# arkworks-rs/marlin

Hardware: NVIDIA H100
Metric: prover_constraints_per_sec (higher is better)
Workload: dtype u32-limb modular integers (Fr 255-bit, Fq 381-bit)

## Files before the change

marlin_b200/csrc/msm.cuh:

```cuda
#pragma once
#include "common.cuh"
#include "curve.cuh"

namespace b2m {

constexpr int MSM_MIN_WINDOW = 8;
constexpr int MSM_BKT_BITS = 24;
constexpr uint32_t MSM_BKT_MASK = (1u << MSM_BKT_BITS) - 1;
constexpr uint32_t MSM_NO_DIGIT = 0xffffffffu;
constexpr int MSM_MAX_BATCH = 8;
constexpr int MSM_MAX_AFFINE_LEVELS = 6;
constexpr size_t MSM_AFFINE_MIN_REFS = (size_t)1 << 23;

template <class Fr, class Fq>
struct MsmJob {
  const Fr* scalars;
  bool mont;
  size_t n;
  size_t base_off;
  const Fr* scalars2;
  size_t n2;
  size_t extra_base;
  const XYZZ<Fq>* extra;
  int n_extra;
  XYZZ<Fq>* out_xyzz;
  Affine<Fq>* out_affine;
  size_t scalar_stride = 1;
};

template <class Fr, class Fq>
struct Msm {
  Ctx* ctx;
  size_t n_srs = 0;
  size_t n_srs_global = 0;
  int tab_rank = 0, tab_world = 1;
  size_t n_extra = 0;
  size_t stride = 0;
  int c = 0, W = 0;
  int affine_levels = Fq::N > 8 ? 3 : 0;
  int affine_ctas_upper = 22;
  int affine_ctas = 4;
  size_t affine_min_refs = MSM_AFFINE_MIN_REFS;
  int affine_map = 1;
  int affine_T = 64;
  int affine_T_upper = 32;
  int acc_ctas_per_sm = 3;
  DBuf<Affine<Fq>> tables;

  static int pick_window(size_t n);
  Msm(Ctx& cx, const Affine<Fq>* powers, size_t n, const Affine<Fq>* host_extra, size_t n_extra_bases, int window_bits,
      bool powers_on_device = false);

  void run(const Fr* scalars, bool mont, size_t n, size_t base_off, const XYZZ<Fq>* extra, int n_extra, XYZZ<Fq>* out_xyzz,
           Affine<Fq>* out_affine);
  void run_batch(const MsmJob<Fr, Fq>* jobs, int nj);
  void run_host(size_t base_off, const uint64_t* scalars, size_t n, uint64_t* out_xy, int* out_is_inf);
  void read_power(size_t i, uint64_t* out_xy);
  static void g1_to_bytes(Ctx& cx, const Affine<Fq>* dev_pts, const uint64_t* host_pts, size_t n, uint8_t* out);
  static void g1_from_bytes(Ctx& cx, const uint8_t* bytes, size_t n, uint64_t* out_xy);
  static void g1_powers_host(Ctx& cx, const uint64_t* g_xy, const uint64_t* beta, size_t n, uint64_t* out);
  static void fixed_base_host(Ctx& cx, const uint64_t* g_xy, const uint64_t* scalars, const uint64_t* beta, size_t first, size_t n, uint64_t* out);
};

}
```

marlin_b200/csrc/msm_affine.cuh:

```cuda
#pragma once
#include "curve.cuh"
#ifdef __CUDACC__
#include "devmem.cuh"
#else
struct uint2 {
  uint32_t x, y;
};
struct uint4 {
  uint32_t x, y, z, w;
};
#endif

namespace b2m {

constexpr uint32_t AFF_BKT_BITS = 24;

template <class Fq>
struct AffLevel {
  const Affine<Fq>* tables;
  size_t table_stride;
  const uint2* sorted;
  const Affine<Fq>* in;
  const uint32_t* off_in;
  const uint32_t* off_out;
  uint32_t B;
  Affine<Fq>* out;
  uint2* out_refs;
  Fq* pref;
  uint4* meta;
  uint32_t T, nthreads;
  uint32_t lane_step;
  Fq* inv;
};

struct AffMap {
  uint32_t o0, step, cnt;
};
template <class Fq>
B2M_HD AffMap aff_map(const AffLevel<Fq>& A, uint32_t t, uint32_t total) {
  AffMap m;
  m.step = A.lane_step;
  uint64_t o0;
  if (A.lane_step == 1) {
    o0 = (uint64_t)t * A.T;
  } else {
    o0 = (uint64_t)(t / A.lane_step) * A.lane_step * A.T + (t % A.lane_step);
  }
  if (o0 >= total) {
    m.o0 = 0;
    m.cnt = 0;
    return m;
  }
  m.o0 = (uint32_t)o0;
  const uint32_t left = (total - m.o0 + m.step - 1) / m.step;
  m.cnt = left < A.T ? left : A.T;
  return m;
}

#if defined(__CUDA_ARCH__)
#define B2M_AFF_LDG(p) ldg_words(p)
#define B2M_AFF_LD(p) ld_words(p)
#define B2M_AFF_ST(p, v) st_words(p, v)
#define B2M_AFF_LDG32(p) __ldg(p)
#else
#define B2M_AFF_LDG(p) (*(p))
#define B2M_AFF_LD(p) (*(p))
#define B2M_AFF_ST(p, v) (*(p) = (v))
#define B2M_AFF_LDG32(p) (*(p))
#endif

B2M_HD uint32_t aff_bucket_of(const uint32_t* off, uint32_t n, uint32_t v) {
  uint32_t lo = 0, hi = n;
  while (hi - lo > 1) {
    uint32_t mid = (lo + hi) >> 1;
    if (B2M_AFF_LDG32(off + mid) <= v) lo = mid; else hi = mid;
  }
  return lo;
}

template <class Fq, bool L0>
B2M_HD void aff_plan_thread(const AffLevel<Fq>& A, uint32_t t) {
  const uint32_t total = B2M_AFF_LDG32(A.off_out + A.B);
  const AffMap mp = aff_map(A, t, total);
  if (!mp.cnt) return;
  uint32_t b = aff_bucket_of(A.off_out, A.B, mp.o0);
  uint32_t b_start = B2M_AFF_LDG32(A.off_out + b), b_end = B2M_AFF_LDG32(A.off_out + b + 1);
  for (uint32_t k = 0; k < mp.cnt; k++) {
    const uint32_t o = mp.o0 + k * mp.step;
    if (o >= b_end) {
      int steps = 0;
      do {
        b++;
        b_end = B2M_AFF_LDG32(A.off_out + b + 1);
      } while (o >= b_end && ++steps < 8);
      if (o >= b_end) {
        b = aff_bucket_of(A.off_out, A.B, o);
        b_end = B2M_AFF_LDG32(A.off_out + b + 1);
      }
      b_start = B2M_AFF_LDG32(A.off_out + b);
    }
    const uint32_t in_start = B2M_AFF_LDG32(A.off_in + b), in_end = B2M_AFF_LDG32(A.off_in + b + 1);
    const uint32_t i0 = in_start + 2u * (o - b_start);
    const bool pair = i0 + 1u < in_end;
    uint4 m;
    if (L0) {
      const uint2 r0 = B2M_AFF_LDG32(A.sorted + i0);
      m.x = (uint32_t)((size_t)(r0.y >> AFF_BKT_BITS) * A.table_stride + (r0.x & 0x7fffffffu)) | (r0.x & 0x80000000u);
      m.y = m.x;
      if (pair) {
        const uint2 r1 = B2M_AFF_LDG32(A.sorted + i0 + 1u);
        m.y = (uint32_t)((size_t)(r1.y >> AFF_BKT_BITS) * A.table_stride + (r1.x & 0x7fffffffu)) | (r1.x & 0x80000000u);
      }
    } else {
      m.x = i0;
      m.y = pair ? i0 + 1u : i0;
    }
    m.z = b;
    m.w = pair ? 1u : 0u;
    A.meta[(size_t)k * A.nthreads + t] = m;
  }
}

template <class Fq>
B2M_HD Fq aff_ldx(const Affine<Fq>* base, uint32_t ref) {
  return B2M_AFF_LDG(&base[ref & 0x7fffffffu].x);
}
template <class Fq>
B2M_HD Affine<Fq> aff_ld(const Affine<Fq>* base, uint32_t ref) {
  const Affine<Fq>* p = base + (ref & 0x7fffffffu);
  Affine<Fq> r;
  r.x = B2M_AFF_LDG(&p->x);
  r.y = B2M_AFF_LDG(&p->y);
  return r;
}
template <class Fq>
B2M_HD Affine<Fq> aff_signed(Affine<Fq> p, uint32_t ref) {
  if (ref >> 31) p.y = p.y.neg();
  return p;
// ... 302 lines not shown
```

marlin_b200/csrc/msm_impl.cuh:

```cuda
#pragma once
#include "msm.cuh"
#include "devmem.cuh"
#include "scan.cuh"
#include "msm_affine.cuh"
#include "comm.cuh"

namespace b2m {

template <class Fq>
__device__ __forceinline__ Affine<Fq> ld_affine(const Affine<Fq>* p) {
  Affine<Fq> r;
  const uint4* q = reinterpret_cast<const uint4*>(p);
  uint32_t* d = reinterpret_cast<uint32_t*>(&r);
#pragma unroll
  for (int i = 0; i < 2 * Fq::N / 4; i++) {
    uint4 v = __ldg(q + i);
    d[4 * i] = v.x; d[4 * i + 1] = v.y; d[4 * i + 2] = v.z; d[4 * i + 3] = v.w;
  }
  return r;
}
template <class Fq> __device__ __noinline__ void g1_add(XYZZ<Fq>& a, const XYZZ<Fq>& b) { a.add(b); }
template <class Fq> __device__ __noinline__ void g1_add_mixed(XYZZ<Fq>& a, const Affine<Fq>& b) { a.add_mixed(b); }
template <class Fq> __device__ __noinline__ void g1_dbl(XYZZ<Fq>& a) { a = a.dbl(); }
template <class Fq> __device__ __noinline__ Fq fq_inverse(const Fq& a) { return a.inverse_fast(); }
template <class Fq> __device__ __noinline__ Affine<Fq> g1_to_affine(const XYZZ<Fq>& p) {
  if (p.is_inf()) return Affine<Fq>::inf();
  Fq izzz = fq_inverse(p.ZZZ);
  Fq izz = (p.ZZ * izzz).sqr();
  return Affine<Fq>{p.X * izz, p.Y * izzz};
}
template <class Fq> __device__ __noinline__ XYZZ<Fq> g1_scalar_mul(const Affine<Fq>& p, const uint32_t* k, int nlimbs) {
  XYZZ<Fq> acc = XYZZ<Fq>::inf();
  bool started = false;
  for (int i = nlimbs - 1; i >= 0; i--) {
    for (int b = 31; b >= 0; b--) {
      if (started) g1_dbl(acc);
      if ((k[i] >> b) & 1u) {
        g1_add_mixed(acc, p);
        started = true;
      }
    }
  }
  return acc;
}

template <class Fq>
__global__ void msm_precompute_kernel(Affine<Fq>* tables, size_t n, int c, int W) {
  size_t i = blockIdx.x * (size_t)blockDim.x + threadIdx.x;
  if (i >= n) return;
  Affine<Fq> cur = ld_affine(tables + i);
  for (int w = 1; w < W; w++) {
    XYZZ<Fq> acc = XYZZ<Fq>::from_affine(cur);
    for (int k = 0; k < c; k++) g1_dbl(acc);
    cur = g1_to_affine(acc);
    st_words(tables + (size_t)w * n + i, cur);
  }
}

template <class Fq>
__global__ void msm_take_residue_kernel(const Affine<Fq>* all, size_t n_loc, int rank, int world, Affine<Fq>* tables) {
  size_t k = blockIdx.x * (size_t)blockDim.x + threadIdx.x;
  if (k >= n_loc) return;
  st_words(tables + k, ld_affine(all + k * (size_t)world + rank));
}

template <class Fr>
__global__ void msm_digits_kernel(const Fr* scalars, size_t sstride, const Fr* scalars2, bool MONT, size_t n, size_t nt, int c, int W,
                                  uint32_t* digits, uint32_t* hist) {
  size_t i = blockIdx.x * (size_t)blockDim.x + threadIdx.x;
  if (i >= nt) return;
  Fr s = i < n ? ld_fr(scalars + i * sstride) : ld_fr(scalars2 + (i - n));
  if (MONT) s = s.to_canonical();
  const uint32_t half = 1u << (c - 1);
  uint32_t carry = 0;
  for (int w = 0; w < W; w++) {
    int bit = w * c;
    int limb = bit >> 5, off = bit & 31;
    uint32_t raw = 0;
    if (limb < Fr::N) {
      raw = s.l[limb] >> off;
      if (off + c > 32 && limb + 1 < Fr::N) raw |= s.l[limb + 1] << (32 - off);
      raw &= (1u << c) - 1;
    }
    uint32_t v = raw + carry;
    uint32_t out;
    if (v > half) {
      uint32_t mag = (1u << c) - v;
      carry = 1;
      out = (mag - 1) | 0x80000000u;
    } else {
      carry = 0;
      out = v ? (v - 1) : MSM_NO_DIGIT;
    }
    digits[(size_t)w * nt + i] = out;
    if (out != MSM_NO_DIGIT) atomicAdd(hist + (out & 0x7fffffffu), 1u);
  }
}


static __global__ void msm_scatter_kernel(const uint32_t* digits, size_t n, size_t nt, size_t base_off, size_t idx2, int W,
                                          uint32_t* cursor, uint2* sorted) {
  size_t i = blockIdx.x * (size_t)blockDim.x + threadIdx.x;
  if (i >= nt) return;
  uint32_t abs_idx = (uint32_t)(i < n ? base_off + i : idx2 + (i - n));
  for (int w = 0; w < W; w++) {
    uint32_t d = digits[(size_t)w * nt + i];
    if (d == MSM_NO_DIGIT) continue;
    uint32_t bkt = d & 0x7fffffffu;
    uint32_t pos = atomicAdd(cursor + bkt, 1u);
    sorted[pos] = make_uint2(abs_idx | (d & 0x80000000u), bkt | ((uint32_t)w << MSM_BKT_BITS));
  }
}

constexpr int MSM_Q = 64;
constexpr int MSM_Q_MIN = 32;
template <class Fq>
__global__ void __launch_bounds__(128)
msm_accumulate_kernel(const Affine<Fq>* __restrict__ tables, size_t table_stride, const uint32_t* __restrict__ offsets,
                      const uint32_t* __restrict__ ends, const uint2* __restrict__ sorted, const uint32_t* __restrict__ total_refs_p,
                      const uint32_t q, XYZZ<Fq>* __restrict__ buckets, XYZZ<Fq>* __restrict__ part_pt,
                      uint32_t* __restrict__ part_bkt) {
  const uint32_t total = *total_refs_p;
  const uint32_t t = blockIdx.x * blockDim.x + threadIdx.x;
  const uint64_t start64 = (uint64_t)t * q;
  uint32_t head_b = MSM_NO_DIGIT, tail_b = MSM_NO_DIGIT;
  if (start64 < total) {
    const uint32_t start = (uint32_t)start64;
    const uint32_t end = (total - start > q) ? start + q : total;
    uint2 rb = __ldg(sorted + start);
    uint32_t ref = rb.x;
    uint32_t cur_b = rb.y & MSM_BKT_MASK;
    uint32_t seg_start = start;
    Affine<Fq> p = ld_affine(tables + (size_t)(rb.y >> MSM_BKT_BITS) * table_stride + (ref & 0x7fffffffu));
    XYZZ<Fq> acc = XYZZ<Fq>::inf();
    for (uint32_t e = start; e < end; e++) {
      Affine<Fq> cur = p;
      const bool neg = ref >> 31;
      uint32_t next_b = cur_b;
      if (e + 1 < end) {
        rb = __ldg(sorted + e + 1);
        ref = rb.x;
        next_b = rb.y & MSM_BKT_MASK;
        p = ld_affine(tables + (size_t)(rb.y >> MSM_BKT_BITS) * table_stride + (ref & 0x7fffffffu));
      }
      acc.add_mixed(cur, neg);
      if (e + 1 == end || next_b != cur_b) {
        const bool whole = (seg_start == offsets[cur_b]) && (e + 1 == ends[cur_b]);
        if (whole) {
          st_words(buckets + cur_b, acc);
        } else if (seg_start == start && head_b == MSM_NO_DIGIT) {
          st_words(part_pt + 2 * (size_t)t, acc);
          head_b = cur_b;
        } else {
          st_words(part_pt + 2 * (size_t)t + 1, acc);
          tail_b = cur_b;
        }
        acc = XYZZ<Fq>::inf();
        seg_start = e + 1;
        cur_b = next_b;
      }
    }
  }
  part_bkt[2 * (size_t)t] = head_b;
  part_bkt[2 * (size_t)t + 1] = tail_b;
}
static __global__ void msm_level_counts_kernel(const uint32_t* off_in, uint32_t B, uint32_t* cnt) {
  uint32_t b = blockIdx.x * blockDim.x + threadIdx.x;
  if (b > B) return;
  cnt[b] = b < B ? (off_in[b + 1] - off_in[b] + 1u) / 2u : 0u;
}
template <class Fq, bool L0>
__global__ void __launch_bounds__(256) msm_affine_plan_kernel(const AffLevel<Fq> A) {
  const uint32_t t = blockIdx.x * blockDim.x + threadIdx.x;
  if (t < A.nthreads) aff_plan_thread<Fq, L0>(A, t);
}
template <class Fq, int MINB, bool PF>
__global__ void __launch_bounds__(128, MINB) msm_affine_level_kernel(const AffLevel<Fq> A, const Affine<Fq>* __restrict__ base) {
  const uint32_t t = blockIdx.x * blockDim.x + threadIdx.x;
  if (t < A.nthreads) aff_level_thread<Fq, PF>(A, base, t);
}

template <class Fq, int MINB, int PHASE, bool PIPE = true>
__global__ void __launch_bounds__(128, MINB) msm_affine_level_sp_kernel(const AffLevel<Fq> A, const Affine<Fq>* __restrict__ base) {
  const uint32_t t = blockIdx.x * blockDim.x + threadIdx.x;
  if (t < A.nthreads) aff_level_thread_sp<Fq, PHASE, PIPE>(A, base, t);
}

template <class Fq>
__device__ __forceinline__ Fq shfl_fq(const Fq& a, int src_lane) {
  Fq r;
#pragma unroll
  for (int i = 0; i < Fq::N; i++) r.l[i] = __shfl_sync(0xffffffffu, a.l[i], src_lane);
  return r;
}
template <class Fq>
__global__ void __launch_bounds__(128) fq_batch_inverse_kernel(Fq* v, size_t n) {
  constexpr int G = 4;
  const size_t t = blockIdx.x * (size_t)blockDim.x + threadIdx.x;
  const int lane = threadIdx.x & 31;
  const size_t i0 = t * G;
  Fq e[G], pre[G];
  Fq run = Fq::one();
#pragma unroll
  for (int k = 0; k < G; k++) {
    e[k] = i0 + k < n ? ld_words(v + i0 + k) : Fq::one();
    pre[k] = run;
    run = run * e[k];
  }
  Fq pin = run, sin = run;
#pragma unroll
  for (int d = 1; d < 32; d <<= 1) {
    const Fq up = shfl_fq(pin, lane - d < 0 ? lane : lane - d);
    const Fq dn = shfl_fq(sin, lane + d > 31 ? lane : lane + d);
    if (lane >= d) pin = pin * up;
    if (lane + d <= 31) sin = sin * dn;
  }
  Fq tinv = Fq::one();
  if (lane == 31) tinv = fq_inverse(pin);
  tinv = shfl_fq(tinv, 31);
  Fq before = shfl_fq(pin, lane == 0 ? 0 : lane - 1), after = shfl_fq(sin, lane == 31 ? 31 : lane + 1);
  if (lane == 0) before = Fq::one();
  if (lane == 31) after = Fq::one();
  Fq inv_run = tinv * before * after;
#pragma unroll
  for (int k = G - 1; k >= 0; k--) {
    const Fq ek = inv_run * pre[k];
    inv_run = inv_run * e[k];
    if (i0 + k < n) st_words(v + i0 + k, ek);
  }
}

struct MsmLongRun {
  uint32_t first, last, bucket;
  uint32_t dst;
};
constexpr uint32_t MSM_RUN_CHUNK = 256;
constexpr uint32_t MSM_RUN_SHORT = 12;
template <class Fq>
__global__ void __launch_bounds__(128)
msm_stitch_kernel(const XYZZ<Fq>* part_pt, const uint32_t* part_bkt, size_t nthreads, const uint32_t q, const uint32_t* offsets,
                  const uint32_t* ends, XYZZ<Fq>* buckets, MsmLongRun* long_runs, MsmLongRun* final_runs, MsmLongRun* short_runs, uint32_t* n_long,
                  uint32_t long_cap, uint32_t chunk_cap) {
  size_t u = blockIdx.x * (size_t)blockDim.x + threadIdx.x;
  if (u >= nthreads) return;
  uint32_t first = 2u * (uint32_t)u + 1u;
  uint32_t b = part_bkt[first];
  if (b == MSM_NO_DIGIT) {
    first = 2u * (uint32_t)u;
    b = part_bkt[first];
    if (b == MSM_NO_DIGIT || offsets[b] != (uint32_t)u * q) return;
  }
  const uint32_t t1 = (ends[b] - 1u) / q;
  const uint32_t last = 2u * t1;
  if (t1 > (uint32_t)u + 1u) {
    const uint32_t nslots = last - first + 1u;
    if (nslots <= MSM_RUN_SHORT) {
      const uint32_t slot = atomicAdd(n_long + 3, 1u);
      if (slot < long_cap) {
        short_runs[slot] = MsmLongRun{first, last, b, MSM_NO_DIGIT};
        return;
      }
    } else if (nslots <= MSM_RUN_CHUNK) {
      const uint32_t slot = atomicAdd(n_long, 1u);
      if (slot < long_cap) {
        long_runs[slot] = MsmLongRun{first, last, b, MSM_NO_DIGIT};
        return;
      }
    } else {
      const uint32_t nch = (nslots + MSM_RUN_CHUNK - 1u) / MSM_RUN_CHUNK;
      const uint32_t c0 = atomicAdd(n_long + 2, nch);
      const uint32_t base = atomicAdd(n_long, nch);
      if (c0 + nch <= chunk_cap && base + nch <= long_cap) {
        for (uint32_t k = 0; k < nch; k++) {
          const uint32_t f = first + k * MSM_RUN_CHUNK;
          const uint32_t l = (last - f >= MSM_RUN_CHUNK) ? f + MSM_RUN_CHUNK - 1u : last;
          long_runs[base + k] = MsmLongRun{f, l, b, c0 + k};
        }
        final_runs[atomicAdd(n_long + 1, 1u)] = MsmLongRun{c0, c0 + nch - 1u, b, MSM_NO_DIGIT};
        return;
      }
      for (uint32_t k = 0; k < nch && base + k < long_cap; k++) long_runs[base + k] = MsmLongRun{1u, 0u, b, MSM_NO_DIGIT};
    }
    XYZZ<Fq> acc = ld_words(part_pt + first);
    for (uint32_t k = first + 1; k <= last; k++)
      if (part_bkt[k] == b) g1_add(acc, ld_words(part_pt + k));
    st_words(buckets + b, acc);
    return;
  }
  XYZZ<Fq> acc = ld_words(part_pt + first);
  g1_add(acc, ld_words(part_pt + last));
  st_words(buckets + b, acc);
}
template <class Fq>
__global__ void __launch_bounds__(128)
msm_stitch_short_kernel(const XYZZ<Fq>* part_pt, const uint32_t* part_bkt, const MsmLongRun* runs, const uint32_t* n_runs, uint32_t cap,
                        XYZZ<Fq>* buckets) {
  uint32_t count = *n_runs;
  if (count > cap) count = cap;
  for (uint32_t r = blockIdx.x * blockDim.x + threadIdx.x; r < count; r += gridDim.x * blockDim.x) {
    const MsmLongRun run = runs[r];
    XYZZ<Fq> acc = ld_words(part_pt + run.first);
    for (uint32_t k = run.first + 1; k <= run.last; k++)
      if (part_bkt[k] == run.bucket) g1_add(acc, ld_words(part_pt + k));
    st_words(buckets + run.bucket, acc);
  }
}
template <class Fq, bool FINAL>
__global__ void __launch_bounds__(128)
msm_stitch_runs_kernel(const XYZZ<Fq>* part_pt, const uint32_t* part_bkt, const MsmLongRun* runs, const uint32_t* n_runs, uint32_t cap,
                       XYZZ<Fq>* buckets, XYZZ<Fq>* chunk_pt) {
  __shared__ uint4 sm_raw[128 * sizeof(XYZZ<Fq>) / 16];
  XYZZ<Fq>* sm = reinterpret_cast<XYZZ<Fq>*>(sm_raw) + (threadIdx.x & ~31u);
  const uint32_t lane = threadIdx.x & 31u;
  uint32_t count = *n_runs;
  if (count > cap) count = cap;
  const uint32_t warps = gridDim.x * (blockDim.x >> 5);
  for (uint32_t r = blockIdx.x * (blockDim.x >> 5) + (threadIdx.x >> 5); r < count; r += warps) {
    const MsmLongRun run = runs[r];
    if (run.first > run.last) continue;
    XYZZ<Fq> acc = XYZZ<Fq>::inf();
    for (uint32_t k = run.first + lane; k <= run.last; k += 32) {
      if (FINAL) g1_add(acc, ld_words(chunk_pt + k));
      else if (part_bkt[k] == run.bucket) g1_add(acc, ld_words(part_pt + k));
    }
    sm[lane] = acc;
    __syncwarp();
    for (uint32_t s2 = 16; s2 >= 1; s2 >>= 1) {
// ... 133 lines not shown
  }
}

template <class Fq>
__global__ void __launch_bounds__(32) msm_combine_kernel(const XYZZ<Fq>* all, int world, int nj, MsmFinishJobs jobs) {
  const int j = blockIdx.x;
  if (threadIdx.x != 0) return;
  XYZZ<Fq> total = XYZZ<Fq>::inf();
  for (int r = 0; r < world; r++) g1_add(total, ld_words(all + (size_t)r * nj + j));
  const XYZZ<Fq>* extra = reinterpret_cast<const XYZZ<Fq>*>(jobs.j[j].extra);
  for (int i = 0; i < jobs.j[j].n_extra; i++) g1_add(total, ld_words(extra + i));
  if (jobs.j[j].out_xyzz) st_words(reinterpret_cast<XYZZ<Fq>*>(jobs.j[j].out_xyzz), total);
  if (jobs.j[j].out_affine) st_words(reinterpret_cast<Affine<Fq>*>(jobs.j[j].out_affine), g1_to_affine(total));
}

constexpr int FB_WIN = 8, FB_WINDOWS = 32, FB_NORM = 16;
template <class Fq>
__global__ void fixed_base_table_kernel(Affine<Fq> g, Affine<Fq>* table) {
  const int t = blockIdx.x * blockDim.x + threadIdx.x;
  if (t >= FB_WINDOWS * 256) return;
  const int k = t >> 8, j = t & 255;
  uint32_t sc[8] = {0, 0, 0, 0, 0, 0, 0, 0};
  sc[k >> 2] = (uint32_t)j << (8 * (k & 3));
  st_words(table + t, j ? g1_to_affine(g1_scalar_mul<Fq>(g, sc, 8)) : Affine<Fq>::inf());
}
template <class Fr, class Fq>
__global__ void __launch_bounds__(128) fixed_base_mul_kernel(const Affine<Fq>* __restrict__ table, const Fr* scalars, Fr beta, size_t first, size_t n,
                                                             XYZZ<Fq>* out) {
  const size_t i = blockIdx.x * (size_t)blockDim.x + threadIdx.x;
  if (i >= n) return;
  const Fr k = scalars ? ld_fr(scalars + i) : beta.pow_u64(first + i).to_canonical();
  XYZZ<Fq> acc = XYZZ<Fq>::inf();
  for (int w = 0; w < FB_WINDOWS && w * FB_WIN < 32 * Fr::N; w++) {
    const uint32_t d = (k.l[w >> 2] >> (8 * (w & 3))) & 255u;
    if (d) g1_add_mixed(acc, ld_affine(table + w * 256 + d));
  }
  st_words(out + i, acc);
}
template <class Fq>
__global__ void __launch_bounds__(128) batch_normalize_kernel(const XYZZ<Fq>* pts, size_t n, Affine<Fq>* out) {
  const size_t t = blockIdx.x * (size_t)blockDim.x + threadIdx.x;
  const size_t i0 = t * FB_NORM;
  if (i0 >= n) return;
  const int cnt = (int)(n - i0 < (size_t)FB_NORM ? n - i0 : FB_NORM);
  Fq pref[FB_NORM];
  Fq run = Fq::one();
  for (int k = 0; k < cnt; k++) {
    const Fq zzz = ld_words(&pts[i0 + k].ZZZ);
    pref[k] = run;
    if (!zzz.is_zero()) run = run * zzz;
  }
  Fq inv = fq_inverse(run);
  for (int k = cnt - 1; k >= 0; k--) {
    const XYZZ<Fq> p = ld_words(pts + i0 + k);
    if (p.is_inf()) {
      st_words(out + i0 + k, Affine<Fq>::inf());
      continue;
    }
    const Fq izzz = inv * pref[k];
    inv = inv * p.ZZZ;
    const Fq izz = (p.ZZ * izzz).sqr();
    st_words(out + i0 + k, Affine<Fq>{p.X * izz, p.Y * izzz});
  }
}

template <class Fq>
__global__ void g1_canonical_kernel(const Affine<Fq>* in, size_t n, Affine<Fq>* out, bool to_bytes) {
  const size_t i = blockIdx.x * (size_t)blockDim.x + threadIdx.x;
  if (i >= n) return;
  Affine<Fq> p = ld_words(in + i);
  if (to_bytes) {
    const bool inf = p.is_inf();
    p.x = p.x.to_canonical();
    p.y = p.y.to_canonical();
    if (inf) p.y.l[Fq::N - 1] |= 1u << 30;
  } else {
    const bool inf = (p.y.l[Fq::N - 1] >> 30) & 1u;
    p.y.l[Fq::N - 1] &= 0x3fffffffu;
    p.x = Fq::from_canonical(p.x);
    p.y = Fq::from_canonical(p.y);
    if (inf) p = Affine<Fq>::inf();
  }
  st_words(out + i, p);
}

template <class Fr, class Fq>
int Msm<Fr, Fq>::pick_window(size_t n) {
  int lg = 0;
  while (((size_t)1 << (lg + 1)) <= n) lg++;
  int c = lg >= 21 ? 20 : (lg >= 17 ? 16 : lg - 1);
  if (c < MSM_MIN_WINDOW) c = MSM_MIN_WINDOW;
  if (c > 20) c = 20;
  auto top_bits = [](int w) {
    const int W = (Fr::Params::BITS + 1 + w - 1) / w;
    return Fr::Params::BITS + 1 - (W - 1) * w;
  };
  if (top_bits(c) < 6) {
    if (c + 1 <= 20 && top_bits(c + 1) >= 6) c = c + 1;
    else if (c - 1 >= MSM_MIN_WINDOW && top_bits(c - 1) >= 6) c = c - 1;
    else if (c - 2 >= MSM_MIN_WINDOW && top_bits(c - 2) >= 6) c = c - 2;
  }
  return c;
}

template <class Fr, class Fq>
Msm<Fr, Fq>::Msm(Ctx& cx, const Affine<Fq>* host_powers, size_t n, const Affine<Fq>* host_extra, size_t n_extra_bases, int window_bits,
                 bool powers_on_device)
    : ctx(&cx), n_extra(n_extra_bases), n_srs_global(n) {
  B2M_REQUIRE(!powers_on_device || cx.world <= 1, B2M_ERR_UNSUPPORTED, "device-resident bases on a multi-GPU context");
  tab_world = cx.world > 1 ? cx.world : 1;
  tab_rank = cx.world > 1 ? cx.rank : 0;
  n_srs = n > (size_t)tab_rank ? (n - tab_rank + tab_world - 1) / tab_world : 0;
  stride = n_srs + n_extra;
  B2M_REQUIRE(n >= 1 && stride < ((size_t)1 << 31), B2M_ERR_INVALID_ARG, "SRS size %zu out of range", n);
  c = window_bits > 0 ? window_bits : pick_window(n / (size_t)tab_world);
  B2M_REQUIRE(c >= MSM_MIN_WINDOW && c <= 24, B2M_ERR_INVALID_ARG, "window bits %d out of range [%d, 24]", c, MSM_MIN_WINDOW);
  W = (Fr::Params::BITS + 1 + c - 1) / c;
  B2M_REQUIRE(W <= 32, B2M_ERR_INVALID_ARG, "too many windows (%d)", W);
  tables = DBuf<Affine<Fq>>(cx, (size_t)W * stride);
  if (powers_on_device) {
    B2M_CUDA(cudaMemcpyAsync(tables.p, host_powers, n * sizeof(Affine<Fq>), cudaMemcpyDeviceToDevice, cx.stream));
  } else if (tab_world == 1) {
    tables.upload(host_powers, n);
  } else if (n_srs) {
    DBuf<Affine<Fq>> all(cx, n);
    all.upload(host_powers, n);
    msm_take_residue_kernel<Fq><<<div_up(n_srs, 256), 256, 0, cx.stream>>>(all.p, n_srs, tab_rank, tab_world, tables.p);
    B2M_CHECK_LAUNCH();
    cx.launches++;
  }
  if (n_extra) B2M_CUDA(cudaMemcpyAsync(tables.p + n_srs, host_extra, n_extra * sizeof(Affine<Fq>), cudaMemcpyHostToDevice, cx.stream));
  if (stride) {
    msm_precompute_kernel<Fq><<<div_up(stride, 128), 128, 0, cx.stream>>>(tables.p, stride, c, W);
    B2M_CHECK_LAUNCH();
    cx.launches++;
  }
  cx.sync();
  B2M_CUDA(cudaOccupancyMaxActiveBlocksPerMultiprocessor(&acc_ctas_per_sm, msm_accumulate_kernel<Fq>, 128, 0));
  if (acc_ctas_per_sm < 1) acc_ctas_per_sm = 1;
  if (const char* e = getenv("B2M_MSM_AFFINE_LEVELS")) affine_levels = atoi(e);
  if (const char* e = getenv("B2M_MSM_AFFINE_T")) affine_T = affine_T_upper = atoi(e);
  if (const char* e = getenv("B2M_MSM_AFFINE_T_UPPER")) affine_T_upper = atoi(e);
  if (const char* e = getenv("B2M_MSM_AFFINE_CTAS")) affine_ctas = atoi(e);
  if (const char* e = getenv("B2M_MSM_AFFINE_CTAS_UPPER")) affine_ctas_upper = atoi(e);
  if (const char* e = getenv("B2M_MSM_AFFINE_MIN_REFS")) affine_min_refs = (size_t)atoll(e);
  if (const char* e = getenv("B2M_MSM_AFFINE_MAP")) affine_map = atoi(e);

  if (affine_levels < 0) affine_levels = 0;
  if (affine_levels > MSM_MAX_AFFINE_LEVELS) affine_levels = MSM_MAX_AFFINE_LEVELS;
  if (affine_T < 1) affine_T = 1;
  if (affine_T > 1024) affine_T = 1024;
  if (affine_T_upper < 1) affine_T_upper = 1;
  if (affine_T_upper > 1024) affine_T_upper = 1024;
}

template <class Fr, class Fq>
void Msm<Fr, Fq>::run(const Fr* scalars, bool mont, size_t n, size_t base_off, const XYZZ<Fq>* extra, int n_extra,
                      XYZZ<Fq>* out_xyzz, Affine<Fq>* out_affine) {
  MsmJob<Fr, Fq> job{scalars, mont, n, base_off, nullptr, 0, 0, extra, n_extra, out_xyzz, out_affine};
  run_batch(&job, 1);
}

template <class Fr, class Fq>
void Msm<Fr, Fq>::run_batch(const MsmJob<Fr, Fq>* jobs_in, int nj) {
  Ctx& cx = *ctx;
  B2M_REQUIRE(nj >= 1 && nj <= MSM_MAX_BATCH, B2M_ERR_INVALID_ARG, "MSM batch of %d jobs", nj);
  MsmJob<Fr, Fq> local[MSM_MAX_BATCH];
  const bool sharded = cx.world > 1;
  B2M_REQUIRE((sharded ? cx.world : 1) == tab_world && (sharded ? cx.rank : 0) == tab_rank, B2M_ERR_INVALID_ARG,
              "this key's tables were built for rank %d of %d; create the SRS after b2m_ctx_attach_comm", tab_rank, tab_world);
  DBuf<XYZZ<Fq>> partial, gathered;
  if (sharded) {
    partial = DBuf<XYZZ<Fq>>(cx, nj);
    gathered = DBuf<XYZZ<Fq>>(cx, (size_t)nj * cx.world);
  }
  for (int j = 0; j < nj; j++) {
    local[j] = jobs_in[j];
    B2M_REQUIRE(jobs_in[j].base_off + jobs_in[j].n <= n_srs_global, B2M_ERR_DEGREE_TOO_LARGE,
                "MSM slice [%zu, %zu) exceeds the SRS (%zu powers)", jobs_in[j].base_off, jobs_in[j].base_off + jobs_in[j].n, n_srs_global);
    if (sharded) {
      const size_t G = (size_t)cx.world, off = jobs_in[j].base_off, n = jobs_in[j].n;
      const size_t skip = ((size_t)cx.rank + G - off % G) % G;
      const size_t cnt = n > skip ? (n - skip + G - 1) / G : 0;
      local[j].scalars = jobs_in[j].scalars + skip;
      local[j].scalar_stride = G;
      local[j].base_off = (off + skip) / G;
      local[j].n = cnt;
      if (cx.rank != 0) { local[j].scalars2 = nullptr; local[j].n2 = 0; }
      local[j].extra = nullptr; local[j].n_extra = 0;
      local[j].out_xyzz = partial.p + j; local[j].out_affine = nullptr;
    }
  }
  const MsmJob<Fr, Fq>* jobs = local;
  size_t max_n = 0;
  for (int j = 0; j < nj; j++) {
    B2M_REQUIRE(jobs[j].n == 0 || jobs[j].base_off + jobs[j].n <= n_srs, B2M_ERR_DEGREE_TOO_LARGE, "MSM slot range [%zu, %zu) exceeds the tables (%zu)",
                jobs[j].base_off, jobs[j].base_off + jobs[j].n, n_srs);
    B2M_REQUIRE(jobs[j].n2 == 0 || jobs[j].extra_base + jobs[j].n2 <= n_extra, B2M_ERR_INVALID_ARG, "extra bases out of range");
    max_n = std::max(max_n, jobs[j].n + jobs[j].n2);
  }
  B2M_REQUIRE((size_t)W * max_n < ((size_t)1 << 32), B2M_ERR_DEGREE_TOO_LARGE, "MSM of %zu pairs x %d windows exceeds 2^32 bucket references", max_n, W);
  MsmFinishJobs fj;
  for (int j = 0; j < nj; j++) fj.j[j] = MsmFinishJob{jobs[j].extra, jobs[j].n_extra, jobs[j].out_xyzz, jobs[j].out_affine};
  auto exchange = [&]() {
    if (!sharded) return;
    size_t spx = cx.span_begin("msm_allgather", (double)nj);
    all_gather_bytes(cx, partial.p, gathered.p, (size_t)nj * sizeof(XYZZ<Fq>));
    MsmFinishJobs oj;
    for (int j = 0; j < nj; j++) oj.j[j] = MsmFinishJob{jobs_in[j].extra, jobs_in[j].n_extra, jobs_in[j].out_xyzz, jobs_in[j].out_affine};
    msm_combine_kernel<Fq><<<nj, 32, 0, cx.stream>>>(gathered.p, cx.world, nj, oj);
    B2M_CHECK_LAUNCH();
    cx.launches++;
    cx.span_end(spx);
  };
  if (max_n == 0) {
    msm_finish_kernel<Fq><<<nj, 64, 0, cx.stream>>>(nullptr, 0, nullptr, 0, 0, fj);
    B2M_CHECK_LAUNCH();
    cx.launches++;
    exchange();
    return;
  }
  const uint32_t B = 1u << (c - 1);
  const int cbits = (c - 1 + 1) / 2, rbits = (c - 1) - cbits;
  const size_t L = (size_t)1 << cbits, R = (size_t)1 << rbits;
  DBuf<XYZZ<Fq>> buckets(cx, (size_t)nj * B);
  {
    const size_t max_refs = (size_t)W * max_n;
    const size_t max_threads = (max_refs + MSM_Q_MIN - 1) / MSM_Q_MIN + 256;
    DBuf<uint32_t> digits[2], hist[2], offsets[2], cursor[2];
    DBuf<uint2> sorted[2];
    const int slots = nj > 1 ? 2 : 1;
    for (int s = 0; s < slots; s++) {
      digits[s] = DBuf<uint32_t>(cx, max_refs); hist[s] = DBuf<uint32_t>(cx, B + 1); offsets[s] = DBuf<uint32_t>(cx, B + 1);
      cursor[s] = DBuf<uint32_t>(cx, B); sorted[s] = DBuf<uint2>(cx, max_refs);
    }
    DBuf<uint32_t> part_bkt(cx, 2 * max_threads), n_long(cx, 4);
    const uint32_t long_cap = 1u << 18;
    const uint32_t chunk_cap = (uint32_t)(4 * max_threads / MSM_RUN_CHUNK + 4);
    DBuf<MsmLongRun> long_runs(cx, long_cap), short_runs(cx, long_cap), final_runs(cx, chunk_cap);
    DBuf<XYZZ<Fq>> chunk_pt(cx, chunk_cap);
    DBuf<XYZZ<Fq>> part_pt(cx, 2 * max_threads);
    const int LV = max_refs >= affine_min_refs ? affine_levels : 0;
    B2M_REQUIRE(LV == 0 || (size_t)W * stride < ((size_t)1 << 31), B2M_ERR_DEGREE_TOO_LARGE,
                "window tables of %d x %zu entries exceed the 31-bit index of the batched-affine plan", W, stride);
    size_t bound[MSM_MAX_AFFINE_LEVELS + 1];
    bound[0] = max_refs;
    for (int l = 1; l <= LV; l++) bound[l] = (bound[l - 1] + B) / 2 + 1;
    DBuf<Affine<Fq>> lvl_pts[2];
    DBuf<uint32_t> lvl_off[2], lvl_cnt;
    DBuf<uint2> lvl_refs;
    DBuf<uint4> lvl_meta;
    DBuf<Fq> lvl_pref, lvl_inv;
    if (LV > 0) {
      lvl_pts[0] = DBuf<Affine<Fq>>(cx, bound[1]);
      if (LV > 1) lvl_pts[1] = DBuf<Affine<Fq>>(cx, bound[2]);
      lvl_off[0] = DBuf<uint32_t>(cx, B + 1); lvl_off[1] = DBuf<uint32_t>(cx, B + 1); lvl_cnt = DBuf<uint32_t>(cx, B + 1);
      lvl_refs = DBuf<uint2>(cx, bound[LV]);
      const size_t T_max = (size_t)std::max(affine_T, affine_T_upper), T_min = (size_t)std::min(affine_T, affine_T_upper);
      const size_t slots_l0 = T_max * ((bound[1] + T_max - 1) / T_max + 128);
      lvl_meta = DBuf<uint4>(cx, slots_l0);
      lvl_pref = DBuf<Fq>(cx, slots_l0);
      lvl_inv = DBuf<Fq>(cx, slots_l0 / T_min + 256);
    }
    buckets.zero();
    cudaEvent_t ev_ready, ev_sorted[MSM_MAX_BATCH], ev_acc[MSM_MAX_BATCH];
    B2M_CUDA(cudaEventCreateWithFlags(&ev_ready, cudaEventDisableTiming));
    for (int j = 0; j < nj; j++) {
      B2M_CUDA(cudaEventCreateWithFlags(&ev_sorted[j], cudaEventDisableTiming));
      B2M_CUDA(cudaEventCreateWithFlags(&ev_acc[j], cudaEventDisableTiming));
    }
    B2M_CUDA(cudaEventRecord(ev_ready, cx.stream));
    B2M_CUDA(cudaStreamWaitEvent(cx.side, ev_ready, 0));
    for (int j = 0; j < nj; j++) {
      const size_t n = jobs[j].n, nt = jobs[j].n + jobs[j].n2;
      const int s = j % slots;
      if (nt == 0) {
        B2M_CUDA(cudaEventRecord(ev_acc[j], cx.stream));
        continue;
      }
      {
        StreamSwap on_side(cx, cx.side);
        if (j >= slots) B2M_CUDA(cudaStreamWaitEvent(cx.side, ev_acc[j - slots], 0));
        hist[s].zero();
        size_t sp0 = cx.span_begin("msm_sort", (double)n);
        msm_digits_kernel<Fr><<<div_up(nt, 256), 256, 0, cx.stream>>>(jobs[j].scalars, jobs[j].scalar_stride, jobs[j].scalars2, jobs[j].mont, n, nt, c, W,
                                                                      digits[s].p, hist[s].p);
        B2M_CHECK_LAUNCH();
        exclusive_scan_u32(cx, hist[s].p, offsets[s].p, B + 1);
        B2M_CUDA(cudaMemcpyAsync(cursor[s].p, offsets[s].p, B * sizeof(uint32_t), cudaMemcpyDeviceToDevice, cx.stream));
        msm_scatter_kernel<<<div_up(nt, 256), 256, 0, cx.stream>>>(digits[s].p, n, nt, jobs[j].base_off, n_srs + jobs[j].extra_base, W,
                                                                    cursor[s].p, sorted[s].p);
        B2M_CHECK_LAUNCH();
        cx.launches += 2;
        cx.span_end(sp0);
        B2M_CUDA(cudaEventRecord(ev_sorted[j], cx.side));
      }
      B2M_CUDA(cudaStreamWaitEvent(cx.stream, ev_sorted[j], 0));
      const Affine<Fq>* src_tables = tables.p;
      size_t src_stride = stride;
      const uint32_t* src_off = offsets[s].p;
      const uint2* src_sorted = sorted[s].p;
      size_t refs = (size_t)W * nt;
      if (LV > 0 && refs >= affine_min_refs) {
        size_t spl = cx.span_begin("msm_affine_levels", (double)n);
        bound[0] = refs;
        for (int l = 1; l <= LV; l++) bound[l] = (bound[l - 1] + B) / 2 + 1;
        const uint32_t* off_in = offsets[s].p;
        for (int l = 0; l < LV; l++) {
          uint32_t* off_out = lvl_off[l & 1].p;
          msm_level_counts_kernel<<<div_up((size_t)B + 1, 256), 256, 0, cx.stream>>>(off_in, B, lvl_cnt.p);
          B2M_CHECK_LAUNCH();
          cx.launches++;
          exclusive_scan_u32(cx, lvl_cnt.p, off_out, (size_t)B + 1);
          const uint32_t lane_step = affine_map ? 32u : 1u;
          const size_t T_l = (size_t)(l == 0 ? affine_T : affine_T_upper);
          const uint32_t nthreads = (uint32_t)(lane_step * ((bound[l + 1] + (size_t)lane_step * T_l - 1) / ((size_t)lane_step * T_l)));
          AffLevel<Fq> A{tables.p, stride, sorted[s].p, l > 0 ? lvl_pts[(l - 1) & 1].p : nullptr, off_in, off_out, B, lvl_pts[l & 1].p,
                         l == LV - 1 ? lvl_refs.p : nullptr, lvl_pref.p, lvl_meta.p, (uint32_t)T_l, nthreads, lane_step, lvl_inv.p};
          if (l == 0)
            msm_affine_plan_kernel<Fq, true><<<div_up(nthreads, 256), 256, 0, cx.stream>>>(A);
          else
            msm_affine_plan_kernel<Fq, false><<<div_up(nthreads, 256), 256, 0, cx.stream>>>(A);
          const Affine<Fq>* base = l == 0 ? tables.p : lvl_pts[(l - 1) & 1].p;
          const unsigned grid = div_up(nthreads, 128);
          const int variant = l == 0 ? affine_ctas : affine_ctas_upper;
          static const char* const lvl_names[MSM_MAX_AFFINE_LEVELS] = {"msm_aff_level0", "msm_aff_level1", "msm_aff_level2", "msm_aff_level3",
                                                                       "msm_aff_level4", "msm_aff_level5"};
          const size_t spk = cx.span_begin(lvl_names[l], (double)n);
          switch (variant) {
            case 3: msm_affine_level_kernel<Fq, 3, true><<<grid, 128, 0, cx.stream>>>(A, base); break;
            case 5: msm_affine_level_kernel<Fq, 5, false><<<grid, 128, 0, cx.stream>>>(A, base); break;
            case 8: msm_affine_level_sp_kernel<Fq, 3, 0><<<grid, 128, 0, cx.stream>>>(A, base); break;
            case 9: msm_affine_level_sp_kernel<Fq, 2, 0><<<grid, 128, 0, cx.stream>>>(A, base); break;
            case 11: case 12: case 13:
              msm_affine_level_sp_kernel<Fq, 5, 1><<<grid, 128, 0, cx.stream>>>(A, base);
              if (variant == 11) msm_affine_level_sp_kernel<Fq, 3, 2><<<grid, 128, 0, cx.stream>>>(A, base);
              else if (variant == 12) msm_affine_level_sp_kernel<Fq, 2, 2><<<grid, 128, 0, cx.stream>>>(A, base);
              else msm_affine_level_sp_kernel<Fq, 4, 2, false><<<grid, 128, 0, cx.stream>>>(A, base);
              cx.launches++;
              break;
            case 21: case 22:
              msm_affine_level_sp_kernel<Fq, 6, 3><<<grid, 128, 0, cx.stream>>>(A, base);
              fq_batch_inverse_kernel<Fq><<<div_up(div_up(nthreads, 4), 128), 128, 0, cx.stream>>>(lvl_inv.p, nthreads);
              if (variant == 21) msm_affine_level_sp_kernel<Fq, 4, 2, false><<<grid, 128, 0, cx.stream>>>(A, base);
              else msm_affine_level_sp_kernel<Fq, 3, 2><<<grid, 128, 0, cx.stream>>>(A, base);
              cx.launches += 2;
              break;
            default: msm_affine_level_kernel<Fq, 4, false><<<grid, 128, 0, cx.stream>>>(A, base); break;
          }
          cx.span_end(spk);
          B2M_CHECK_LAUNCH();
          cx.launches += 2;
          off_in = off_out;
        }
        cx.span_end(spl);
        src_tables = lvl_pts[(LV - 1) & 1].p;
        src_stride = 0;
        src_off = off_in;
        src_sorted = lvl_refs.p;
        refs = bound[LV];
      }
      const uint32_t* src_ends = src_off + 1;
      const uint32_t* src_total = src_off + B;
      size_t sp = cx.span_begin("msm_accumulate_kernel", (double)n);
      const size_t wave = (size_t)cx.sm_count * acc_ctas_per_sm * 128;
      size_t waves = (refs + wave * MSM_Q / 2) / (wave * MSM_Q);
      if (waves < 1) waves = 1;
      uint32_t q = (uint32_t)((refs + waves * wave - 1) / (waves * wave));
      if (q < (uint32_t)MSM_Q_MIN) q = MSM_Q_MIN;
      const size_t nthreads = (refs + q - 1) / q;
      msm_accumulate_kernel<Fq><<<div_up(nthreads, 128), 128, 0, cx.stream>>>(src_tables, src_stride, src_off, src_ends, src_sorted,
                                                                               src_total, q, buckets.p + (size_t)j * B, part_pt.p,
                                                                               part_bkt.p);
      B2M_CHECK_LAUNCH();
      cx.launches++;
      cx.span_end(sp);
      size_t sp1 = cx.span_begin("msm_stitch", (double)n);
      n_long.zero();
      msm_stitch_kernel<Fq><<<div_up(nthreads, 128), 128, 0, cx.stream>>>(part_pt.p, part_bkt.p, nthreads, q, src_off, src_ends,
                                                                           buckets.p + (size_t)j * B, long_runs.p, final_runs.p, short_runs.p, n_long.p,
                                                                           long_cap, chunk_cap);
      msm_stitch_short_kernel<Fq><<<2 * cx.sm_count, 128, 0, cx.stream>>>(part_pt.p, part_bkt.p, short_runs.p, n_long.p + 3, long_cap,
                                                                          buckets.p + (size_t)j * B);
      msm_stitch_runs_kernel<Fq, false><<<4 * cx.sm_count, 128, 0, cx.stream>>>(part_pt.p, part_bkt.p, long_runs.p, n_long.p, long_cap,
                                                                                buckets.p + (size_t)j * B, chunk_pt.p);
      msm_stitch_runs_kernel<Fq, true><<<cx.sm_count, 128, 0, cx.stream>>>(part_pt.p, part_bkt.p, final_runs.p, n_long.p + 1, chunk_cap,
                                                                           buckets.p + (size_t)j * B, chunk_pt.p);
      B2M_CHECK_LAUNCH();
      cx.launches += 4;
      cx.span_end(sp1);
      B2M_CUDA(cudaEventRecord(ev_acc[j], cx.stream));
    }
    cudaEventDestroy(ev_ready);
    for (int j = 0; j < nj; j++) {
      cudaEventDestroy(ev_sorted[j]);
      cudaEventDestroy(ev_acc[j]);
    }
  }
  double units = 0;
  for (int j = 0; j < nj; j++) units += (double)jobs[j].n;
  size_t sp2 = cx.span_begin("msm_reduce", units);
  DBuf<XYZZ<Fq>> rsum(cx, (size_t)nj * R), csum(cx, (size_t)nj * L);
  {
    const uint32_t Kr = (uint32_t)std::min<size_t>(L, 8), Kc = (uint32_t)std::min<size_t>(R, 8);
    const size_t seg_r = L / Kr, seg_c = R / Kc;
    DBuf<XYZZ<Fq>> part_r(cx, (size_t)nj * R * seg_r), part_c(cx, (size_t)nj * L * seg_c);
    msm_segsum_kernel<Fq><<<div_up((size_t)nj * R * seg_r, 128), 128, 0, cx.stream>>>(buckets.p, part_r.p, (size_t)nj, seg_r, Kr, R, 1, L, B);
    msm_segsum_kernel<Fq><<<div_up((size_t)nj * L * seg_c, 128), 128, 0, cx.stream>>>(buckets.p, part_c.p, (size_t)nj, seg_c, Kc, L, L, 1, B);
    const MsmFoldJob fr{part_r.p, rsum.p, (size_t)nj * R, seg_r}, fc{part_c.p, csum.p, (size_t)nj * L, seg_c};
    msm_fold_kernel<Fq><<<div_up(((size_t)nj * R + (size_t)nj * L) * 32, 128), 128, 0, cx.stream>>>(fr, fc);
    B2M_CHECK_LAUNCH();
    cx.launches += 3;
  }
  DBuf<XYZZ<Fq>> rplanes(cx, (size_t)nj * (rbits + 1)), cplanes(cx, (size_t)nj * (cbits + 1));
  msm_bitplane_kernel<Fq><<<dim3(rbits + 1 + cbits + 1, nj), 256, 0, cx.stream>>>(rsum.p, R, rbits, rplanes.p, csum.p, L, cbits, cplanes.p);
  B2M_CHECK_LAUNCH();
  cx.launches++;
  msm_finish_kernel<Fq><<<nj, 64, 0, cx.stream>>>(rplanes.p, rbits, cplanes.p, cbits, 1, fj);
  B2M_CHECK_LAUNCH();
  cx.launches++;
  cx.span_end(sp2);
  exchange();
}

template <class Fr, class Fq>
void Msm<Fr, Fq>::run_host(size_t base_off, const uint64_t* scalars, size_t n, uint64_t* out_xy, int* out_is_inf) {
  Ctx& cx = *ctx;
  DBuf<Fr> sc(cx, n ? n : 1);
  if (n) sc.upload(reinterpret_cast<const Fr*>(scalars), n);
  DBuf<Affine<Fq>> res(cx, 1);
  run(sc.p, false, n, base_off, nullptr, 0, nullptr, res.p);
  Affine<Fq> h;
  res.download(&h, 1);
  memcpy(out_xy, &h, sizeof(h));
  if (out_is_inf) *out_is_inf = h.is_inf() ? 1 : 0;
}

template <class Fr, class Fq>
void Msm<Fr, Fq>::read_power(size_t i, uint64_t* out_xy) {
  B2M_REQUIRE(i < n_srs_global, B2M_ERR_INVALID_ARG, "power %zu of %zu", i, n_srs_global);
  B2M_REQUIRE(tab_world == 1, B2M_ERR_UNSUPPORTED, "read_power on a sharded key (the power lives on rank %zu)", i % (size_t)tab_world);
  Affine<Fq> h;
  B2M_CUDA(cudaMemcpyAsync(&h, tables.p + i, sizeof(h), cudaMemcpyDeviceToHost, ctx->stream));
  ctx->sync();
  memcpy(out_xy, &h, sizeof(h));
}

template <class Fr, class Fq>
void Msm<Fr, Fq>::fixed_base_host(Ctx& cx, const uint64_t* g_xy, const uint64_t* scalars, const uint64_t* beta, size_t first, size_t n, uint64_t* out) {
  Affine<Fq> g;
  memcpy(&g, g_xy, sizeof(g));
  Fr b = Fr::zero();
  if (beta) {
    memcpy(&b, beta, sizeof(b));
    b = Fr::from_canonical(b);
  }
  if (n == 0) return;
  DBuf<Affine<Fq>> table(cx, FB_WINDOWS * 256);
  fixed_base_table_kernel<Fq><<<div_up(FB_WINDOWS * 256, 64), 64, 0, cx.stream>>>(g, table.p);
  B2M_CHECK_LAUNCH();
  cx.launches++;
  const size_t slice = (size_t)1 << 22;
// ... 51 lines not shown
```

Measured before the change: 4.113 million.

## Size MSM affine-level and accumulate grids to whole occupancy waves, derive chain length on device

Affine levels now launch a thread count that is a whole multiple of one occupancy wave, with the wave size taken from the kernels' reported max active blocks. The per-thread chain length is computed on the device from the actual ref total rather than an upper bound, and the nominal affine_T is raised. The accumulate and stitch kernels likewise take a fixed wave-aligned thread count and derive refs-per-thread from the device-side total. The aim is to remove tail-wave imbalance and idle threads that come from sizing grids by worst-case bounds. In exchange, meta and prefix buffers are sized per level and each thread may get a longer chain.

Result: faster. 4.209 million, median of 6 (+2.3%).

```diff
diff --git a/marlin_b200/csrc/msm.cuh b/marlin_b200/csrc/msm.cuh
--- a/marlin_b200/csrc/msm.cuh
+++ b/marlin_b200/csrc/msm.cuh
@@ -42,12 +42,16 @@
   int affine_ctas = 4;
   size_t affine_min_refs = MSM_AFFINE_MIN_REFS;
   int affine_map = 1;
-  int affine_T = 64;
+  int affine_T = 128;
   int affine_T_upper = 32;
+  bool affine_T_exact = false, affine_T_upper_exact = false;
+  int affine_wave_ctas = 4, affine_wave_ctas_upper = 6;
   int acc_ctas_per_sm = 3;
   DBuf<Affine<Fq>> tables;
 
   static int pick_window(size_t n);
+  void level_grid(int level, size_t bound, uint32_t lane_step, uint32_t* nthreads, uint32_t* T) const;
+  size_t acc_threads(size_t refs) const;
   Msm(Ctx& cx, const Affine<Fq>* powers, size_t n, const Affine<Fq>* host_extra, size_t n_extra_bases, int window_bits,
       bool powers_on_device = false);
 
diff --git a/marlin_b200/csrc/msm_affine.cuh b/marlin_b200/csrc/msm_affine.cuh
--- a/marlin_b200/csrc/msm_affine.cuh
+++ b/marlin_b200/csrc/msm_affine.cuh
@@ -31,20 +31,28 @@
   uint32_t T, nthreads;
   uint32_t lane_step;
   Fq* inv;
+  uint32_t derive_T;
 };
 
 struct AffMap {
   uint32_t o0, step, cnt;
 };
 template <class Fq>
+B2M_HD uint32_t aff_chain_len(const AffLevel<Fq>& A, uint32_t total) {
+  if (!A.derive_T || total == 0) return A.T;
+  const uint32_t T = (total - 1u) / A.nthreads + 1u;
+  return T < A.T ? T : A.T;
+}
+template <class Fq>
 B2M_HD AffMap aff_map(const AffLevel<Fq>& A, uint32_t t, uint32_t total) {
   AffMap m;
   m.step = A.lane_step;
+  const uint32_t T = aff_chain_len(A, total);
   uint64_t o0;
   if (A.lane_step == 1) {
-    o0 = (uint64_t)t * A.T;
+    o0 = (uint64_t)t * T;
   } else {
-    o0 = (uint64_t)(t / A.lane_step) * A.lane_step * A.T + (t % A.lane_step);
+    o0 = (uint64_t)(t / A.lane_step) * A.lane_step * T + (t % A.lane_step);
   }
   if (o0 >= total) {
     m.o0 = 0;
@@ -53,7 +61,7 @@
   }
   m.o0 = (uint32_t)o0;
   const uint32_t left = (total - m.o0 + m.step - 1) / m.step;
-  m.cnt = left < A.T ? left : A.T;
+  m.cnt = left < T ? left : T;
   return m;
 }
 
diff --git a/marlin_b200/csrc/msm_impl.cuh b/marlin_b200/csrc/msm_impl.cuh
--- a/marlin_b200/csrc/msm_impl.cuh
+++ b/marlin_b200/csrc/msm_impl.cuh
@@ -1,4 +1,5 @@
 #pragma once
+#include <numeric>
 #include "msm.cuh"
 #include "devmem.cuh"
 #include "scan.cuh"
@@ -114,13 +115,17 @@
 
 constexpr int MSM_Q = 64;
 constexpr int MSM_Q_MIN = 32;
+__device__ __forceinline__ uint32_t msm_refs_per_thread(uint32_t total, uint32_t nthreads) {
+  return total ? (total - 1u) / nthreads + 1u : 1u;
+}
 template <class Fq>
 __global__ void __launch_bounds__(128)
 msm_accumulate_kernel(const Affine<Fq>* __restrict__ tables, size_t table_stride, const uint32_t* __restrict__ offsets,
                       const uint32_t* __restrict__ ends, const uint2* __restrict__ sorted, const uint32_t* __restrict__ total_refs_p,
-                      const uint32_t q, XYZZ<Fq>* __restrict__ buckets, XYZZ<Fq>* __restrict__ part_pt,
+                      const uint32_t nthreads, XYZZ<Fq>* __restrict__ buckets, XYZZ<Fq>* __restrict__ part_pt,
                       uint32_t* __restrict__ part_bkt) {
   const uint32_t total = *total_refs_p;
+  const uint32_t q = msm_refs_per_thread(total, nthreads);
   const uint32_t t = blockIdx.x * blockDim.x + threadIdx.x;
   const uint64_t start64 = (uint64_t)t * q;
   uint32_t head_b = MSM_NO_DIGIT, tail_b = MSM_NO_DIGIT;
@@ -238,11 +243,12 @@
 constexpr uint32_t MSM_RUN_SHORT = 12;
 template <class Fq>
 __global__ void __launch_bounds__(128)
-msm_stitch_kernel(const XYZZ<Fq>* part_pt, const uint32_t* part_bkt, size_t nthreads, const uint32_t q, const uint32_t* offsets,
+msm_stitch_kernel(const XYZZ<Fq>* part_pt, const uint32_t* part_bkt, uint32_t nthreads, const uint32_t* total_refs_p, const uint32_t* offsets,
                   const uint32_t* ends, XYZZ<Fq>* buckets, MsmLongRun* long_runs, MsmLongRun* final_runs, MsmLongRun* short_runs, uint32_t* n_long,
                   uint32_t long_cap, uint32_t chunk_cap) {
   size_t u = blockIdx.x * (size_t)blockDim.x + threadIdx.x;
   if (u >= nthreads) return;
+  const uint32_t q = msm_refs_per_thread(*total_refs_p, nthreads);
   uint32_t first = 2u * (uint32_t)u + 1u;
   uint32_t b = part_bkt[first];
   if (b == MSM_NO_DIGIT) {
@@ -542,6 +548,33 @@
     if (inf) p = Affine<Fq>::inf();
   }
   st_words(out + i, p);
+}
+
+template <class Fq>
+static int level_wave_ctas(int variant) {
+  auto occ = [](auto kernel) {
+    int ctas = 0;
+    B2M_CUDA(cudaOccupancyMaxActiveBlocksPerMultiprocessor(&ctas, kernel, 128, 0));
+    return ctas < 1 ? 1 : ctas;
+  };
+  int a = 0, b = 0;
+  switch (variant) {
+    case 3: a = occ(msm_affine_level_kernel<Fq, 3, true>); break;
+    case 5: a = occ(msm_affine_level_kernel<Fq, 5, false>); break;
+    case 8: a = occ(msm_affine_level_sp_kernel<Fq, 3, 0>); break;
+    case 9: a = occ(msm_affine_level_sp_kernel<Fq, 2, 0>); break;
+    case 11: case 12: case 13:
+      a = occ(msm_affine_level_sp_kernel<Fq, 5, 1>);
+      b = variant == 11 ? occ(msm_affine_level_sp_kernel<Fq, 3, 2>)
+                        : variant == 12 ? occ(msm_affine_level_sp_kernel<Fq, 2, 2>) : occ(msm_affine_level_sp_kernel<Fq, 4, 2, false>);
+      break;
+    case 21: case 22:
+      a = occ(msm_affine_level_sp_kernel<Fq, 6, 3>);
+      b = variant == 21 ? occ(msm_affine_level_sp_kernel<Fq, 4, 2, false>) : occ(msm_affine_level_sp_kernel<Fq, 3, 2>);
+      break;
+    default: a = occ(msm_affine_level_kernel<Fq, 4, false>); break;
+  }
+  return b ? a / std::gcd(a, b) * b : a;
 }
 
 template <class Fr, class Fq>
@@ -599,8 +632,14 @@
   B2M_CUDA(cudaOccupancyMaxActiveBlocksPerMultiprocessor(&acc_ctas_per_sm, msm_accumulate_kernel<Fq>, 128, 0));
   if (acc_ctas_per_sm < 1) acc_ctas_per_sm = 1;
   if (const char* e = getenv("B2M_MSM_AFFINE_LEVELS")) affine_levels = atoi(e);
-  if (const char* e = getenv("B2M_MSM_AFFINE_T")) affine_T = affine_T_upper = atoi(e);
-  if (const char* e = getenv("B2M_MSM_AFFINE_T_UPPER")) affine_T_upper = atoi(e);
+  if (const char* e = getenv("B2M_MSM_AFFINE_T")) {
+    affine_T = affine_T_upper = atoi(e);
+    affine_T_exact = affine_T_upper_exact = true;
+  }
+  if (const char* e = getenv("B2M_MSM_AFFINE_T_UPPER")) {
+    affine_T_upper = atoi(e);
+    affine_T_upper_exact = true;
+  }
   if (const char* e = getenv("B2M_MSM_AFFINE_CTAS")) affine_ctas = atoi(e);
   if (const char* e = getenv("B2M_MSM_AFFINE_CTAS_UPPER")) affine_ctas_upper = atoi(e);
   if (const char* e = getenv("B2M_MSM_AFFINE_MIN_REFS")) affine_min_refs = (size_t)atoll(e);
@@ -612,6 +651,33 @@
   if (affine_T > 1024) affine_T = 1024;
   if (affine_T_upper < 1) affine_T_upper = 1;
   if (affine_T_upper > 1024) affine_T_upper = 1024;
+  if (affine_levels > 0) {
+    affine_wave_ctas = level_wave_ctas<Fq>(affine_ctas);
+    affine_wave_ctas_upper = level_wave_ctas<Fq>(affine_ctas_upper);
+  }
+}
+
+template <class Fr, class Fq>
+void Msm<Fr, Fq>::level_grid(int l, size_t bound, uint32_t lane_step, uint32_t* nthreads, uint32_t* T) const {
+  const size_t T_nom = (size_t)(l == 0 ? affine_T : affine_T_upper);
+  if (l == 0 ? affine_T_exact : affine_T_upper_exact) {
+    *T = (uint32_t)T_nom;
+    *nthreads = (uint32_t)(lane_step * ((bound + (size_t)lane_step * T_nom - 1) / ((size_t)lane_step * T_nom)));
+    return;
+  }
+  const size_t wave = (size_t)ctx->sm_count * (l == 0 ? affine_wave_ctas : affine_wave_ctas_upper) * 128;
+  size_t k = (bound + wave * T_nom / 2) / (wave * T_nom);
+  if (k < 1) k = 1;
+  *nthreads = (uint32_t)(k * wave);
+  const size_t t = (bound + k * wave - 1) / (k * wave);
+  *T = (uint32_t)(t ? t : 1);
+}
+
+template <class Fr, class Fq>
+size_t Msm<Fr, Fq>::acc_threads(size_t refs) const {
+  const size_t wave = (size_t)ctx->sm_count * acc_ctas_per_sm * 128;
+  if (refs < wave * MSM_Q_MIN) return std::max<size_t>(128, div_up(div_up(refs, (size_t)MSM_Q_MIN), (size_t)128) * 128);
+  return std::max<size_t>(1, (refs + wave * MSM_Q / 2) / (wave * MSM_Q)) * wave;
 }
 
 template <class Fr, class Fq>
@@ -686,7 +752,11 @@
   DBuf<XYZZ<Fq>> buckets(cx, (size_t)nj * B);
   {
     const size_t max_refs = (size_t)W * max_n;
-    const size_t max_threads = (max_refs + MSM_Q_MIN - 1) / MSM_Q_MIN + 256;
+    const int LV = max_refs >= affine_min_refs ? affine_levels : 0;
+    size_t bound[MSM_MAX_AFFINE_LEVELS + 1];
+    bound[0] = max_refs;
+    for (int l = 1; l <= LV; l++) bound[l] = (bound[l - 1] + B) / 2 + 1;
+    const size_t max_threads = acc_threads(std::max(max_refs, bound[LV]));
     DBuf<uint32_t> digits[2], hist[2], offsets[2], cursor[2];
     DBuf<uint2> sorted[2];
     const int slots = nj > 1 ? 2 : 1;
@@ -700,27 +770,29 @@
     DBuf<MsmLongRun> long_runs(cx, long_cap), short_runs(cx, long_cap), final_runs(cx, chunk_cap);
     DBuf<XYZZ<Fq>> chunk_pt(cx, chunk_cap);
     DBuf<XYZZ<Fq>> part_pt(cx, 2 * max_threads);
-    const int LV = max_refs >= affine_min_refs ? affine_levels : 0;
     B2M_REQUIRE(LV == 0 || (size_t)W * stride < ((size_t)1 << 31), B2M_ERR_DEGREE_TOO_LARGE,
                 "window tables of %d x %zu entries exceed the 31-bit index of the batched-affine plan", W, stride);
-    size_t bound[MSM_MAX_AFFINE_LEVELS + 1];
-    bound[0] = max_refs;
-    for (int l = 1; l <= LV; l++) bound[l] = (bound[l - 1] + B) / 2 + 1;
     DBuf<Affine<Fq>> lvl_pts[2];
     DBuf<uint32_t> lvl_off[2], lvl_cnt;
     DBuf<uint2> lvl_refs;
     DBuf<uint4> lvl_meta;
     DBuf<Fq> lvl_pref, lvl_inv;
+    const uint32_t lane_step = affine_map ? 32u : 1u;
     if (LV > 0) {
       lvl_pts[0] = DBuf<Affine<Fq>>(cx, bound[1]);
       if (LV > 1) lvl_pts[1] = DBuf<Affine<Fq>>(cx, bound[2]);
       lvl_off[0] = DBuf<uint32_t>(cx, B + 1); lvl_off[1] = DBuf<uint32_t>(cx, B + 1); lvl_cnt = DBuf<uint32_t>(cx, B + 1);
       lvl_refs = DBuf<uint2>(cx, bound[LV]);
-      const size_t T_max = (size_t)std::max(affine_T, affine_T_upper), T_min = (size_t)std::min(affine_T, affine_T_upper);
-      const size_t slots_l0 = T_max * ((bound[1] + T_max - 1) / T_max + 128);
-      lvl_meta = DBuf<uint4>(cx, slots_l0);
-      lvl_pref = DBuf<Fq>(cx, slots_l0);
-      lvl_inv = DBuf<Fq>(cx, slots_l0 / T_min + 256);
+      size_t slots = 1, inv_slots = 1;
+      for (int l = 0; l < LV; l++) {
+        uint32_t nth, T_l;
+        level_grid(l, bound[l + 1], lane_step, &nth, &T_l);
+        slots = std::max(slots, ((size_t)T_l + 1) * nth);
+        inv_slots = std::max(inv_slots, (size_t)nth);
+      }
+      lvl_meta = DBuf<uint4>(cx, slots);
+      lvl_pref = DBuf<Fq>(cx, slots);
+      lvl_inv = DBuf<Fq>(cx, inv_slots);
     }
     buckets.zero();
     cudaEvent_t ev_ready, ev_sorted[MSM_MAX_BATCH], ev_acc[MSM_MAX_BATCH];
@@ -772,11 +844,11 @@
           B2M_CHECK_LAUNCH();
           cx.launches++;
           exclusive_scan_u32(cx, lvl_cnt.p, off_out, (size_t)B + 1);
-          const uint32_t lane_step = affine_map ? 32u : 1u;
-          const size_t T_l = (size_t)(l == 0 ? affine_T : affine_T_upper);
-          const uint32_t nthreads = (uint32_t)(lane_step * ((bound[l + 1] + (size_t)lane_step * T_l - 1) / ((size_t)lane_step * T_l)));
+          uint32_t nthreads, T_l;
+          level_grid(l, bound[l + 1], lane_step, &nthreads, &T_l);
+          const uint32_t derive_T = (l == 0 ? affine_T_exact : affine_T_upper_exact) ? 0u : 1u;
           AffLevel<Fq> A{tables.p, stride, sorted[s].p, l > 0 ? lvl_pts[(l - 1) & 1].p : nullptr, off_in, off_out, B, lvl_pts[l & 1].p,
-                         l == LV - 1 ? lvl_refs.p : nullptr, lvl_pref.p, lvl_meta.p, (uint32_t)T_l, nthreads, lane_step, lvl_inv.p};
+                         l == LV - 1 ? lvl_refs.p : nullptr, lvl_pref.p, lvl_meta.p, T_l, nthreads, lane_step, lvl_inv.p, derive_T};
           if (l == 0)
             msm_affine_plan_kernel<Fq, true><<<div_up(nthreads, 256), 256, 0, cx.stream>>>(A);
           else
@@ -823,21 +895,16 @@
       const uint32_t* src_ends = src_off + 1;
       const uint32_t* src_total = src_off + B;
       size_t sp = cx.span_begin("msm_accumulate_kernel", (double)n);
-      const size_t wave = (size_t)cx.sm_count * acc_ctas_per_sm * 128;
-      size_t waves = (refs + wave * MSM_Q / 2) / (wave * MSM_Q);
-      if (waves < 1) waves = 1;
-      uint32_t q = (uint32_t)((refs + waves * wave - 1) / (waves * wave));
-      if (q < (uint32_t)MSM_Q_MIN) q = MSM_Q_MIN;
-      const size_t nthreads = (refs + q - 1) / q;
-      msm_accumulate_kernel<Fq><<<div_up(nthreads, 128), 128, 0, cx.stream>>>(src_tables, src_stride, src_off, src_ends, src_sorted,
-                                                                               src_total, q, buckets.p + (size_t)j * B, part_pt.p,
-                                                                               part_bkt.p);
+      const uint32_t nthreads = (uint32_t)acc_threads(refs);
+      msm_accumulate_kernel<Fq><<<nthreads / 128, 128, 0, cx.stream>>>(src_tables, src_stride, src_off, src_ends, src_sorted,
+                                                                        src_total, nthreads, buckets.p + (size_t)j * B, part_pt.p,
+                                                                        part_bkt.p);
       B2M_CHECK_LAUNCH();
       cx.launches++;
       cx.span_end(sp);
       size_t sp1 = cx.span_begin("msm_stitch", (double)n);
       n_long.zero();
-      msm_stitch_kernel<Fq><<<div_up(nthreads, 128), 128, 0, cx.stream>>>(part_pt.p, part_bkt.p, nthreads, q, src_off, src_ends,
+      msm_stitch_kernel<Fq><<<div_up(nthreads, 128), 128, 0, cx.stream>>>(part_pt.p, part_bkt.p, nthreads, src_total, src_off, src_ends,
                                                                            buckets.p + (size_t)j * B, long_runs.p, final_runs.p, short_runs.p, n_long.p,
                                                                            long_cap, chunk_cap);
       msm_stitch_short_kernel<Fq><<<2 * cx.sm_count, 128, 0, cx.stream>>>(part_pt.p, part_bkt.p, short_runs.p, n_long.p + 3, long_cap,
```
